# fverdoja/Fast-3D-Pointcloud-Segmentation

Hardware: AMD Instinct MI355X
Metric: Mpoints/sec segmented end-to-end, 1M-pt RGB-D frames (higher is better)
Workload: dtype f32

## Files before the change

__graft_entry__.py:

```python
import importlib
import os
import subprocess
import sys

ROOT = os.path.dirname(os.path.abspath(__file__))
PKG = "fast-3d-pointcloud-segmentation_amd"


def _run(cmd):
    print("+", " ".join(cmd), flush=True)
    subprocess.run(cmd, check=True)


def build() -> None:
    _run(["make", "-C", os.path.join(ROOT, PKG, "csrc")])
    _run(["make", "-C", os.path.join(ROOT, "oracle")])
    _run(["make", "-C", os.path.join(ROOT, "tests", "emul")])
    _run(["make", "-C", os.path.join(ROOT, "tests", "devprobe")])
    _run(["make", "-C", os.path.join(ROOT, "tests", "kernprobe")])
    _run(["make", "-C", os.path.join(ROOT, "tests", "blockprobe")])
    if ROOT not in sys.path:
        sys.path.insert(0, ROOT)
    P = importlib.import_module(PKG)
    lib = P.load_library()
    assert lib.f3ds_version() >= 120
    P.check_library_is_current(lib)


def smoke() -> None:
    import ctypes
    import numpy as np
    if ROOT not in sys.path:
        sys.path.insert(0, ROOT)
    sys.path.insert(0, os.path.join(ROOT, "tests"))
    P = importlib.import_module(PKG)
    from conftest import CpuChecker
    if P.device_count() < 1:
        raise RuntimeError("smoke(): no HIP device visible; libf3ds has no CPU fallback")
    pts = P.synth_frame(0, 7, 160, 120, 30)
    prm = P.launch_params(voxel_res=0.02, seed_res=0.2)
    ctx = P.Context(0)
    labels = ctx.segment(pts, prm)
    ora = CpuChecker(os.path.join(ROOT, "oracle", "libf3ds_oracle.so"), "f3ds_oracle")
    rc, olabels, ores, oh = ora.segment(pts, prm)
    assert rc == 0
    assert np.array_equal(labels, olabels), "HIP labels differ from the oracle"
    assert ctx.result.n_regions == ores.n_regions and ctx.result.n_merges == ores.n_merges
    print("smoke ok: N=%d V=%d S=%d E=%d merges=%d regions=%d  (%.2f ms on device 0)" % (
        len(pts), ctx.result.n_voxels, ctx.result.n_supervoxels, ctx.result.n_edges, ctx.result.n_merges, ctx.result.n_regions, ctx.result.ms_total))
    ctx.close()


if __name__ == "__main__":
    build()
    if len(sys.argv) > 1 and sys.argv[1] == "smoke":
        smoke()
```

fast-3d-pointcloud-segmentation_amd/__init__.py:

```python
import ctypes
import os

import numpy as np

_HERE = os.path.dirname(os.path.abspath(__file__))
def _dev_env(name):
    return os.environ.get(name) if os.environ.get("F3DS_DEV", "0") not in ("", "0") else None


LIB_PATH = _dev_env("F3DS_LIB") or os.path.join(_HERE, "libf3ds.so")

NO_LABEL = 0xFFFFFFFF
LAB_CIEDE00, RGB_EUCL = 0, 1
NORMALS_DIFF, CONVEX_NORMALS_DIFF = 0, 1
MANUAL_LAMBDA, ADAPTIVE_LAMBDA, EQUALIZATION = 0, 1, 2
DEPTH_U16, DEPTH_F32 = 0, 1
COLOR_RGB8, COLOR_RGBA8, COLOR_PACKED = 0, 1, 2

DBG = dict(GRID=0, VOXEL_KEYS=1, VOXEL_COUNT=2, VOXEL_XYZ=3, VOXEL_RGB=4, VOXEL_NORMAL=5, VOXEL_NEIGHBORS=6,
           POINT_VOXEL=7, SEED_ORIG=8, SEED_KEPT=9, VOXEL_SVLABEL=10, VOXEL_DIST=11, SV_LABELS=12, SV_CENTROID=13,
           EDGES=14, EDGE_DELTAS=15, EDGE_WEIGHTS=16, MERGES=17, VOXEL_REGION=18, SV_REGION=19)
DBG_INFO = dict(MERGE_LAYOUT=20, TILE_LIST_LEN=21, SWEEP_STATS=22, STAGE0_PATH=23, LAUNCH_SHAPE=24)
DBG_CLOUD_PATH = 25
DBG_DTYPE = dict(GRID=np.float64, VOXEL_KEYS=np.uint32, VOXEL_COUNT=np.uint32, VOXEL_XYZ=np.float32, VOXEL_RGB=np.float32,
                 VOXEL_NORMAL=np.float32, VOXEL_NEIGHBORS=np.int32, POINT_VOXEL=np.int32, SEED_ORIG=np.int32, SEED_KEPT=np.int32,
                 VOXEL_SVLABEL=np.uint32, VOXEL_DIST=np.float32, SV_LABELS=np.uint32, SV_CENTROID=np.float32, EDGES=np.uint32,
                 EDGE_DELTAS=np.float32, EDGE_WEIGHTS=np.float32, MERGES=np.uint32, VOXEL_REGION=np.uint32, SV_REGION=np.uint32)


class F3dsError(RuntimeError):
    def __init__(self, code, text):
        super().__init__("f3ds error %d: %s" % (code, text))
        self.code = code


class LogicError(F3dsError):
    """std::logic_error of the reference (clustering.cpp:576,591,671)."""


class Params(ctypes.Structure):
    _fields_ = [("voxel_res", ctypes.c_float), ("seed_res", ctypes.c_float), ("w_color", ctypes.c_float),
                ("w_spatial", ctypes.c_float), ("w_normal", ctypes.c_float), ("use_transform", ctypes.c_int32),
                ("color_metric", ctypes.c_int32), ("geom_metric", ctypes.c_int32), ("merging", ctypes.c_int32),
                ("lambda_", ctypes.c_float), ("bins", ctypes.c_int32), ("threshold", ctypes.c_float),
                ("leaf_order", ctypes.c_int32), ("fold_negative_z", ctypes.c_int32)]

    def copy(self):
        p = Params()
        ctypes.memmove(ctypes.byref(p), ctypes.byref(self), ctypes.sizeof(Params))
        return p


class Result(ctypes.Structure):
    _fields_ = [("n_points", ctypes.c_uint64), ("n_finite", ctypes.c_uint64), ("n_voxels", ctypes.c_uint32),
                ("octree_depth", ctypes.c_uint32), ("n_seed_cells", ctypes.c_uint32), ("n_seeds", ctypes.c_uint32),
                ("n_supervoxels", ctypes.c_uint32), ("n_edges", ctypes.c_uint32), ("n_merges", ctypes.c_uint32),
                ("n_regions", ctypes.c_uint32), ("sweeps", ctypes.c_uint32), ("lambda_", ctypes.c_float),
                ("ms_total", ctypes.c_float), ("ms_stage", ctypes.c_float * 8)]

    def as_dict(self):
        d = {k: getattr(self, k) for k, _ in self._fields_ if k != "ms_stage"}
        d["ms_stage"] = list(self.ms_stage)
        return d


class RgbdFormat(ctypes.Structure):
    _fields_ = [("width", ctypes.c_uint32), ("height", ctypes.c_uint32), ("depth_type", ctypes.c_int32), ("depth_scale", ctypes.c_float),
                ("color_format", ctypes.c_int32), ("depth_pitch", ctypes.c_uint32), ("color_pitch", ctypes.c_uint32),
                ("fx", ctypes.c_float), ("fy", ctypes.c_float), ("cx", ctypes.c_float), ("cy", ctypes.c_float)]

    def copy(self):
        f = RgbdFormat()
        ctypes.memmove(ctypes.byref(f), ctypes.byref(self), ctypes.sizeof(RgbdFormat))
        return f


# ... 952 lines not shown
        return self._get("region_adjacency", [_PAIR])[0]

    def cluster_supervoxels(self, sv, adjacency_pairs, params):
        a = {k: np.ascontiguousarray(sv[k], np.float32 if k in ("voxel_xyz", "centroid_xyz", "normal") else np.uint32) for k in
             ("label", "voxel_offset", "voxel_xyz", "voxel_rgba", "centroid_xyz", "normal")}
        S = len(a["label"])
        if a["voxel_offset"].shape != (S + 1,):
            raise ValueError("voxel_offset must hold n_supervoxels + 1 = %d entries, has shape %s" % (S + 1, a["voxel_offset"].shape))
        nvox = int(a["voxel_offset"][S])
        if a["voxel_xyz"].size != 3 * nvox or a["voxel_rgba"].size != nvox:
            raise ValueError("voxel_xyz / voxel_rgba must hold voxel_offset[-1] = %d voxels (have %d / %d)" % (nvox, a["voxel_xyz"].size // 3, a["voxel_rgba"].size))
        if a["centroid_xyz"].size != 3 * S or a["normal"].size != 3 * S:
            raise ValueError("centroid_xyz and normal must have shape (%d, 3)" % S)
        st = SupervoxelSet(S, *[a[k].ctypes.data for k in ("label", "voxel_offset", "voxel_xyz", "voxel_rgba", "centroid_xyz", "normal")])
        pairs = np.ascontiguousarray(adjacency_pairs, np.uint32).reshape(-1, 2)
        region = np.zeros(S, np.uint32); vlab = np.zeros(nvox, np.uint32)
        _check(self.lib, self.lib.f3ds_cluster_supervoxels(self.handle, ctypes.byref(st), pairs.ctypes.data, len(pairs), ctypes.byref(params), region.ctypes.data,
                                                           vlab.ctypes.data, ctypes.byref(self.result)))
        self._n = nvox
        return region, vlab

    def regions(self):
        return dict(zip(("label", "n_voxels", "xyz", "normal", "rgb"), self._get("regions", [_U32, _U32, _XYZ, _XYZ, _XYZ])))

    def region_voxels(self):
        return tuple(self._get("region_voxels", [_XYZ, _U32, _U32]))

    def voxel_cloud(self):
        return tuple(self._get("voxel_cloud", [_XYZ, _U32, _U32]))

    def merge_layout(self):
        nb = ctypes.c_size_t(); buf = np.zeros(2, np.uint32)
        _check(self.lib, self.lib.f3ds_get_debug(self.handle, 20, buf.ctypes.data, 8, ctypes.byref(nb)))
        return int(buf[0]), int(buf[1])

    def stage0_path(self):
        nb = ctypes.c_size_t(); buf = np.zeros(1, np.uint32)
        _check(self.lib, self.lib.f3ds_get_debug(self.handle, 23, buf.ctypes.data, 4, ctypes.byref(nb)))
        return "tiles" if buf[0] else "sort"

    def launch_shape(self):
        nb = ctypes.c_size_t(); buf = np.zeros(3, np.uint32)
        _check(self.lib, self.lib.f3ds_get_debug(self.handle, DBG_INFO["LAUNCH_SHAPE"], buf.ctypes.data, 12, ctypes.byref(nb)))
        return tuple(int(x) for x in buf)

    def sweep_stats(self):
        nb = ctypes.c_size_t(); buf = np.zeros(4, np.uint32)
        _check(self.lib, self.lib.f3ds_get_debug(self.handle, 22, buf.ctypes.data, 16, ctypes.byref(nb)))
        return tuple(int(x) for x in buf)

    def tile_list_lengths(self):
        return self._get("debug", [(np.uint8, ())], DBG_INFO["TILE_LIST_LEN"])[0].view(np.uint32)

    def debug(self, name):
        return self._get("debug", [(np.uint8, ())], DBG[name])[0].view(DBG_DTYPE[name])


class FrameStream(_Handle):

    _destroy = "f3ds_stream_destroy"

    def __init__(self, device=0, depth=8, groups=0):
        self.lib = load_library()
        h = ctypes.c_void_p()
        _check(self.lib, self.lib.f3ds_stream_create(device, depth, groups, ctypes.byref(h)))
        self.handle = h
        self.depth = depth

    def __enter__(self):
        return self

    def __exit__(self, *exc):
        self.close()

    def pending(self):
        return self.lib.f3ds_stream_pending(self.handle)

    def buffer(self, n):
        p = ctypes.c_void_p()
        rc = self.lib.f3ds_stream_buffer(self.handle, n, ctypes.byref(p))
        if rc == ERR_BUSY:
            return None
        _check(self.lib, rc)
        return np.ctypeslib.as_array(ctypes.cast(p, ctypes.POINTER(ctypes.c_float)), shape=(max(n, 1), 4))[:n]

    def submit(self, points, params, tag=0):
        pts = np.ascontiguousarray(points, np.float32).reshape(-1, 4)
        rc = self.lib.f3ds_stream_submit(self.handle, pts.ctypes.data, len(pts), ctypes.byref(params), tag)
        if rc == ERR_BUSY:
            return False
        _check(self.lib, rc)
        return True

    def submit_rgbd(self, depth, color, fmt, params, tag=0):
        f, d, c = _rgbd_images(fmt, depth, color)
        rc = self.lib.f3ds_stream_submit_rgbd(self.handle, ctypes.byref(f), d.ctypes.data, c.ctypes.data, ctypes.byref(params), tag)
        if rc == ERR_BUSY:
            return False
        _check(self.lib, rc)
        return True

    def next(self, wait=True):
        n = ctypes.c_size_t(); tag = ctypes.c_uint64(); res = Result()
        probe = np.empty(1, np.uint32)
        rc = self.lib.f3ds_stream_next(self.handle, probe.ctypes.data, 0, ctypes.byref(n), ctypes.byref(tag), ctypes.byref(res), 1 if wait else 0)
        if rc in (ERR_EMPTY, ERR_BUSY):
# ... 687 lines not shown
```

fast-3d-pointcloud-segmentation_amd/csrc/f3ds_algo.h:

```cpp
#ifndef F3DS_ALGO_H_
#define F3DS_ALGO_H_

#include "f3ds_numerics.h"

namespace f3ds {

#define F3DS_MAX_SEED_EVENTS 48
struct SeedEvent {
    int trigger;
    int depth;
    double min[3];
    unsigned off[3];
};
struct SeedGrid {
    int n_events;
    int error;
    int defined;
    int depth;
    double res;
    double min[3], max[3];
    unsigned off[3];
    SeedEvent ev[F3DS_MAX_SEED_EVENTS];
};
F3DS_HD void a_seed_init(SeedGrid& g, float seed_res) {
// ... 455 lines not shown
    rec[0] = acc[6] / c; rec[1] = acc[7] / c; rec[2] = acc[8] / c;
    float n4[4];
    n_plane_normal(acc, count, rec, n4);
    rec[3] = n4[0]; rec[4] = n4[1]; rec[5] = n4[2];
    rec[6] = acc[9]; rec[7] = acc[10]; rec[8] = acc[11];
    n_rgb2lab(rec + 6, rec + 9);
    rec[12] = rec[13] = rec[14] = rec[15] = 0.0f;
}

struct MergeParams {
    int color_metric, geom_metric, merging;
    float lambda;
    int bins;
    const float* cdf_c;
    const float* cdf_g;
};
F3DS_HD float a_tc(const MergeParams& p, float dc, int* err) {
    if (p.merging != 2) return p.lambda * dc;
    short bin = (short)__builtin_floorf(dc * (float)(short)p.bins);
    if (bin == (short)p.bins) bin--;
    if (bin < 0 || bin >= (short)p.bins) { *err = -9; return 0.0f; }
    return p.cdf_c[bin] / 2;
}
F3DS_HD float a_tg(const MergeParams& p, float dg, int* err) {
    if (p.merging != 2) return (1 - p.lambda) * dg;
    short bin = (short)__builtin_floorf(dg * (float)(short)p.bins);
    if (bin < 0 || bin >= (short)p.bins) { *err = -9; return 0.0f; }
    return p.cdf_g[bin] / 2;
}
template <class K = m_lit> F3DS_HD float a_edge_weight(const MergeParams& p, const float* rec_first, const float* rec_second, int* err, K mc = K()) {
    float dc, dg;
    n_delta_c_g(rec_first, rec_second, p.color_metric, p.geom_metric, &dc, &dg, mc);
    return a_tc(p, dc, err) + a_tg(p, dg, err);
}

struct EdgeHist {
    const uint32_t* ev_epoch;
    const uint32_t* ev_key;
    const int* ev_prev;
};
F3DS_HD bool a_edge_before(const EdgeHist& H, uint32_t e, uint32_t ke, int he, uint32_t f, uint32_t kf, int hf) {
    if (ke != kf) return ke < kf;
    for (;;) {
        uint32_t te = H.ev_epoch[he], tf = H.ev_epoch[hf];
        uint32_t tau = te > tf ? te : tf;
        if (tau == 0u) return e < f;
        if (te == tau) he = H.ev_prev[he];
        if (tf == tau) hf = H.ev_prev[hf];
        ke = H.ev_key[he]; kf = H.ev_key[hf];
        if (ke != kf) return ke < kf;
    }
}

}
#endif
```

fast-3d-pointcloud-segmentation_amd/csrc/f3ds_hip.hip:

```cpp
#include <hip/hip_runtime.h>

#include <algorithm>
#include <cmath>
#include <atomic>
#include <map>
#include <chrono>
#include <cstdio>
#include <cstdlib>
#include <cstring>
#include <string>
#include <type_traits>
#include <mutex>
#include <set>
#include <vector>

#include "../../include/f3ds.h"
#include "f3ds_algo.h"
#include "f3ds_glasbey.h"
#include "f3ds_eval.h"
#include "f3ds_dev.h"
#include "f3ds_levels.h"
#include "f3ds_eval_levels.h"
#include "f3ds_rgbd.h"
#include "f3ds_label_image.h"
// ... 1668 lines not shown
}

extern "C" int f3ds_get_supervoxels(f3ds_ctx* c, uint32_t* label, float* xyz, float* rgb, float* normal, uint32_t* n_voxels, size_t cap, size_t* n_out) {
    if (const int frc = on_frame(c)) return frc;
    return supervoxels_of(c, c->hcount, c->hc, label, xyz, rgb, normal, n_voxels, cap, n_out);
}

extern "C" int f3ds_get_supervoxel_adjacency(f3ds_ctx* c, uint32_t* pairs, size_t cap_pairs, size_t* n_out) {
    if (const int frc = on_frame(c)) return frc;
    const uint32_t E = c->E;
    int rc;
    if (!all_fit(E, cap_pairs, pairs != nullptr, n_out, &rc)) return rc;
    std::vector<uint32_t> a, b;
    if ((rc = fetch(c, c->ea0, E, a)) || (rc = fetch(c, c->eb0, E, b))) return rc;
    for (uint32_t e = 0; e < E; ++e) { pairs[2 * e] = label_out(c, a[e]); pairs[2 * e + 1] = label_out(c, b[e]); }
    return F3DS_OK;
}

extern "C" int f3ds_get_region_adjacency(f3ds_ctx* c, uint32_t* pairs, size_t cap_pairs, size_t* n_out) {
    if (const int frc = on_frame(c)) return frc;
    std::vector<uint32_t> a, b, root;
    int rc;
    if ((rc = fetch(c, c->ea0, c->E, a)) || (rc = fetch(c, c->eb0, c->E, b)) || (rc = fetch(c, c->root, c->S0 + 1, root))) return rc;
    std::vector<uint64_t> keys;
    for (uint32_t e = 0; e < c->E; ++e) {
        const uint32_t p = root[a[e]], q = root[b[e]];
        if (p != q) keys.push_back(((uint64_t)(p < q ? p : q) << 32) | (p < q ? q : p));
    }
    std::sort(keys.begin(), keys.end());
    keys.erase(std::unique(keys.begin(), keys.end()), keys.end());
    if (!all_fit(keys.size(), cap_pairs, pairs != nullptr, n_out, &rc)) return rc;
    for (size_t k = 0; k < keys.size(); ++k) { pairs[2 * k] = label_out(c, (uint32_t)(keys[k] >> 32)); pairs[2 * k + 1] = label_out(c, (uint32_t)keys[k]); }
    return F3DS_OK;
}

extern "C" int f3ds_merge_layout_info(uint32_t n_edges, int waves, int keys_in_lds, uint32_t out[4]) {
    if (!out || (waves != 4 && waves != 8) || (keys_in_lds != 0 && keys_in_lds != 2)) return F3DS_ERR_ARG;
    const MergeIlLayout L = merge_il_offsets(n_edges, waves, keys_in_lds);
    out[0] = L.total; out[1] = L.sp_rows; out[2] = L.Ecap;
    out[3] = (L.total <= MC_LDS_LIMIT && (uint64_t)n_edges * (keys_in_lds == 2 ? 10u : 2u) <= (1u << 22)) ? 1u : 0u;
    return F3DS_OK;
}
extern "C" int f3ds_get_debug(f3ds_ctx* c, int what, void* dst, size_t cap_bytes, size_t* bytes_out) {
    if (const int frc = on_frame(c, NEED_NOTHING)) return frc;
    const uint32_t V = c->V, S0 = c->S0, E = c->E, n = c->n;
    std::vector<uint8_t> buf;
    auto put = [&](const void* src, size_t nb) { const uint8_t* b = static_cast<const uint8_t*>(src); buf.insert(buf.end(), b, b + nb); };
    int rc = F3DS_OK;
    std::vector<float> f; std::vector<uint32_t> u, u2, u3; std::vector<int> iv; std::vector<unsigned char> uc;
    if (what != F3DS_DBG_GRID && what != F3DS_DBG_LAUNCH_SHAPE && what != F3DS_DBG_CLOUD_PATH && !c->have_frame) return F3DS_ERR_LOGIC;
    switch (what) {
        case F3DS_DBG_GRID: { HIPCHECK(hipMemcpy(c->h_grid, c->d_grid, sizeof(GridInfo), hipMemcpyDeviceToHost)); double g[5] = {c->h_grid->min[0], c->h_grid->min[1], c->h_grid->min[2], c->h_grid->res, (double)c->h_grid->depth}; put(g, sizeof g); break; }
        case F3DS_DBG_TILE_LIST_LEN: if ((rc = fetch(c, c->tile_n1, (size_t)(V + NT_TILE - 1) / NT_TILE, u))) return rc; put(u.data(), u.size() * 4); break;
        case F3DS_DBG_LAUNCH_SHAPE: put(c->launch_shape, 12); break;
        case F3DS_DBG_CLOUD_PATH: put(&c->cloud_path, 4); break;
        case F3DS_DBG_STAGE0_PATH: { const uint32_t w = c->vox_hashed ? 1u : 0u; put(&w, 4); break; }
        case F3DS_DBG_SWEEP_STATS: {
            DevCounters dcs;
            HIPCHECK(hipMemcpy(&dcs, c->d_dc, sizeof dcs, hipMemcpyDeviceToHost));
            put(dcs.sweep_stats, 16);
#ifdef F3DS_CEN_STATS
            fprintf(stderr, "d_centroid: quads %u, live rows %u, to the wave path: list %u, leaves %u; per quad ndmax %.2f, max leaves %.1f; per row nd %.2f, leaves %.1f\n", dcs.cen_stats[0], dcs.cen_stats[1], dcs.cen_stats[2],
                    dcs.cen_stats[3], dcs.cen_stats[4] / (double)dcs.cen_stats[0], dcs.cen_stats[7] / (double)dcs.cen_stats[0], dcs.cen_stats[5] / (double)dcs.cen_stats[1], dcs.cen_stats[6] / (double)dcs.cen_stats[1]);
#endif
            break;
        }
        case F3DS_DBG_MERGE_LAYOUT: { const uint32_t w[2] = {c->merge_kind == MK_GLOBAL ? 0u : (uint32_t)mk_waves(c->merge_kind), c->merge_kind == MK_GLOBAL ? 0u : (uint32_t)mk_res(c->merge_kind)}; put(w, 8); break; }
        case F3DS_DBG_VOXEL_KEYS: if ((rc = fetch(c, c->vkey, (size_t)V * 3, u))) return rc; put(u.data(), u.size() * 4); break;
        case F3DS_DBG_VOXEL_COUNT: if ((rc = fetch(c, c->vcount, V, u))) return rc; put(u.data(), u.size() * 4); break;
        case F3DS_DBG_VOXEL_XYZ: case F3DS_DBG_VOXEL_RGB: case F3DS_DBG_VOXEL_NORMAL:
            if ((rc = fetch(c, c->vf, (size_t)V * 12, f))) return rc;
            for (uint32_t v = 0; v < V; ++v) {
                if (what == F3DS_DBG_VOXEL_XYZ) put(&f[(size_t)v * 12], 12);
                else if (what == F3DS_DBG_VOXEL_RGB) put(&f[(size_t)v * 12 + 3], 12);
                else { float n4[4] = {f[(size_t)v * 12 + 6], f[(size_t)v * 12 + 7], f[(size_t)v * 12 + 8], 0.0f}; put(n4, 16); }
            }
            break;
        case F3DS_DBG_VOXEL_NEIGHBORS: if ((rc = fetch(c, c->nbr, (size_t)V * 27, iv))) return rc; put(iv.data(), iv.size() * 4); break;
        case F3DS_DBG_POINT_VOXEL: if ((rc = fetch(c, c->pt_voxel, n, iv))) return rc; put(iv.data(), iv.size() * 4); break;
        case F3DS_DBG_SEED_ORIG: if ((rc = fetch(c, c->seed_orig, c->C, iv))) return rc; put(iv.data(), iv.size() * 4); break;
        case F3DS_DBG_SEED_KEPT: if ((rc = fetch(c, c->seed_kept, S0, iv))) return rc; put(iv.data(), iv.size() * 4); break;
        case F3DS_DBG_VOXEL_SVLABEL: if ((rc = fetch(c, c->owner0, V, u))) return rc; put(u.data(), u.size() * 4); break;
        case F3DS_DBG_VOXEL_DIST: if ((rc = fetch(c, c->dist0, V, f))) return rc; put(f.data(), f.size() * 4); break;
        case F3DS_DBG_SV_LABELS: case F3DS_DBG_SV_CENTROID: case F3DS_DBG_SV_REGION:
            if ((rc = fetch(c, c->hcount, S0 + 1, u)) || (rc = fetch(c, c->hc, (size_t)(S0 + 1) * 12, f)) || (rc = fetch(c, c->root, S0 + 1, u2))) return rc;
            for (uint32_t h = 1; h <= S0; ++h) {
                if (!u[h]) continue;
                const uint32_t lh = label_out(c, h), lr = label_out(c, u2[h]);
                if (what == F3DS_DBG_SV_LABELS) put(&lh, 4);
                else if (what == F3DS_DBG_SV_REGION) put(&lr, 4);
                else { float r[10]; for (int k = 0; k < 9; ++k) r[k] = f[(size_t)h * 12 + k]; r[9] = 0.0f; put(r, 40); }
            }
            break;
        case F3DS_DBG_EDGES:
            if ((rc = fetch(c, c->ea0, E, u)) || (rc = fetch(c, c->eb0, E, u2))) return rc;
            for (uint32_t e = 0; e < E; ++e) { const uint32_t la = label_out(c, u[e]), lb = label_out(c, u2[e]); put(&la, 4); put(&lb, 4); }
            break;
        case F3DS_DBG_EDGE_DELTAS: if ((rc = fetch(c, c->deltas, (size_t)E * 2, f))) return rc; put(f.data(), f.size() * 4); break;
        case F3DS_DBG_EDGE_WEIGHTS: {
            if ((rc = fetch(c, c->deltas, (size_t)E * 2, f))) return rc;
            MergeParams mp; mp.color_metric = c->prm.color_metric; mp.geom_metric = c->prm.geom_metric; mp.merging = c->prm.merging;
            mp.lambda = c->res.lambda; mp.bins = (c->prm.merging == F3DS_EQUALIZATION && c->prm.bins != 0) ? (short)c->prm.bins : 500;
            std::vector<float> cdf;
            if (c->prm.merging == F3DS_EQUALIZATION) { if ((rc = fetch(c, c->cdf, (size_t)2 * mp.bins, cdf))) return rc; mp.cdf_c = cdf.data(); mp.cdf_g = cdf.data() + mp.bins; }
            else { mp.cdf_c = mp.cdf_g = nullptr; }
            for (uint32_t e = 0; e < E; ++e) { int err = 0; float w = a_tc(mp, f[e * 2], &err) + a_tg(mp, f[e * 2 + 1], &err); put(&w, 4); }
// ... 1067 lines not shown
```

fast-3d-pointcloud-segmentation_amd/csrc/f3ds_kernels.inc:

```


namespace {

struct P16 { float x, y, z; uint32_t rgba; };

struct DevCounters {
    unsigned long long n_finite;
    uint32_t bbox[6];
    uint32_t bbox_any;
    uint32_t n_valid;
    uint32_t n_voxels;
    uint32_t n_cells;
    uint32_t n_seeds;
    uint32_t n_edges;
    uint32_t n_alive;
    uint32_t n_merges;
    uint32_t n_regions;
    uint32_t n_events;
    int error;
    int r_overflow;
    float lambda;
    uint32_t seg_count;
    uint32_t n_ghosts;
    int depth;
// ... 1044 lines not shown
constexpr int SW_SLOT_BITS = 9;
constexpr int SW_SLOT_WORDS = (27 * SW_SLOT_BITS + 31) / 32;
static_assert(NT_RING1 < (1 << SW_SLOT_BITS), "a list position must fit its bit field");
__device__ __forceinline__ void sw_slots_pack(const uint32_t pos[27], uint32_t w[SW_SLOT_WORDS]) {
#pragma unroll
    for (int k = 0; k < SW_SLOT_WORDS; ++k) w[k] = 0u;
#pragma unroll
    for (int j = 0; j < 27; ++j) {
        const int bit = j * SW_SLOT_BITS, wi = bit >> 5, sh = bit & 31;
        w[wi] |= pos[j] << sh;
        if (sh + SW_SLOT_BITS > 32) w[wi + 1] |= pos[j] >> (32 - sh);
    }
}
__device__ __forceinline__ uint32_t sw_slot(const uint32_t w[SW_SLOT_WORDS], int j) {
    const int bit = j * SW_SLOT_BITS, wi = bit >> 5, sh = bit & 31;
    uint32_t x = w[wi] >> sh;
    if (sh + SW_SLOT_BITS > 32) x |= w[wi + 1] << (32 - sh);
    return x & ((1u << SW_SLOT_BITS) - 1u);
}
__device__ inline void cov_add(float acc[9], const float4 q) {
    acc[0] += q.x * q.x; acc[1] += q.x * q.y; acc[2] += q.x * q.z;
    acc[3] += q.y * q.y; acc[4] += q.y * q.z; acc[5] += q.z * q.z;
    acc[6] += q.x; acc[7] += q.y; acc[8] += q.z;
}
__device__ __forceinline__ uint32_t lds_addr(const float* p);
typedef float f3ds_f2 __attribute__((ext_vector_type(2)));
typedef float f3ds_f4 __attribute__((ext_vector_type(4)));
struct CovPairs {
    f3ds_f2 a0, a1, a2, a3; float sz;
    __device__ void zero() { a0 = a1 = a2 = a3 = f3ds_f2{0.0f, 0.0f}; sz = 0.0f; }
    __device__ void add(const f3ds_f4 q) {
        const f3ds_f2 xy = q.xy, zy = q.zw;
        a0 += xy * q.xx;
        a1 += xy * q.zz;
        a2 += zy * zy;
        a3 += xy;
        sz += q.z;
    }
    __device__ void store(float acc[9]) const { acc[0] = a0.x; acc[1] = a0.y; acc[2] = a1.x; acc[3] = a2.y; acc[4] = a1.y; acc[5] = a2.x; acc[6] = a3.x; acc[7] = a3.y; acc[8] = sz; }
};
template <int NTT>
struct d_normals_t {
    static constexpr int BLOCK = NTT;
    static constexpr int PT = (NT_RING1 * 27 + NTT - 1) / NTT;
    static constexpr int PR = PT % 9 == 0 ? 9 : (PT % 8 == 0 ? 8 : (PT % 6 == 0 ? 6 : (PT % 4 == 0 ? 4 : (PT % 3 == 0 ? 3 : (PT % 2 == 0 ? 2 : 1)))));
#ifndef F3DS_NORMALS_WPS
#define F3DS_NORMALS_WPS 3
#endif
#ifndef F3DS_NORMALS_WPS256
#define F3DS_NORMALS_WPS256 3
#endif
    static constexpr int WAVES_PER_SIMD = NTT > 256 ? F3DS_NORMALS_WPS : F3DS_NORMALS_WPS256;
    __device__ static uint32_t hslot(uint32_t ord) { return (ord * 2654435761u) >> 21; }
    __device__ void one_tile(const uint32_t bix, float* vf, const int* nbr, const DevCounters* dc, uint32_t* tile_n1, uint32_t* tile_ord, uint32_t* tile_slots, uint32_t holes) const {
        __shared__ uint32_t hw[NT_HCAP];
        __shared__ __attribute__((aligned(16))) float4 xyz[NT_SLOTS + 1];
        __shared__ uint32_t sord[NT_SLOTS];
        __shared__ uint16_t rows[NT_RING1 + 1][28];
        __shared__ uint32_t n_slots, overflow;
        __shared__ uint16_t tme[NT_TILE];
        const uint32_t KB = lds_addr(reinterpret_cast<const float*>(xyz)) >> 4;
        const uint32_t V = dc->n_voxels;
        const uint32_t v0 = bix * NT_TILE;
        if (v0 >= V) return;
        const uint32_t nt = V - v0 < (uint32_t)NT_TILE ? V - v0 : (uint32_t)NT_TILE;
#ifdef F3DS_MERGE_PROF
        unsigned long long tp[8], tq = __builtin_amdgcn_s_memtime(); int tpi = 0;
        unsigned long long tx_[12] = {0, 0, 0, 0, 0, 0, 0, 0, 0, 0, 0, 0}, tq2 = tq;
#define NPH() do { const unsigned long long n_ = __builtin_amdgcn_s_memtime(); tp[tpi++] = n_ - tq; tq = n_; } while (0)
#define NPX(i) do { const unsigned long long n_ = __builtin_amdgcn_s_memtime(); tx_[i] = n_ - tq2; tq2 = n_; } while (0)
#else
#define NPH() do { } while (0)
#define NPX(i) do { } while (0)
#endif
        for (int i = threadIdx.x; i < NT_HCAP; i += NTT) hw[i] = 0u;
        if (threadIdx.x == 0) { n_slots = 0; overflow = V >= NT_ORD_LIMIT ? 1u : 0u; xyz[NT_ZERO] = make_float4(0.0f, 0.0f, 0.0f, 0.0f); }
        __syncthreads();
        auto insert_key_from = [&](uint32_t ord, uint32_t h, uint32_t old) -> uint32_t {
            for (int probes = 0; probes < NT_HCAP; ++probes) {
                if (old == 0u) old = atomicCAS(&hw[h], 0u, ((ord + 1u) << 10) | NT_HNONE);
                if (old == 0u || (old >> 10) == ord + 1u) return h;
                h = (h + 1u) & (NT_HCAP - 1);
                old = hw[h];
            }
            overflow = 1;
            return 0u;
        };
        auto lookup = [&](uint32_t ord) -> uint16_t {
            uint32_t h = hslot(ord);
            for (;;) {
                const uint32_t k = hw[h];
                if ((k >> 10) == ord + 1u) return (k & NT_HNONE) == NT_HNONE ? NT_NONE : (uint16_t)(k & NT_HNONE);
                if (k == 0u) return NT_NONE;
                h = (h + 1u) & (NT_HCAP - 1);
            }
        };
        NPH();
        {
            constexpr int R1 = (NT_TILE * 27 + NTT - 1) / NTT;
            int u1[R1];
#pragma unroll
            for (int j = 0; j < R1; ++j) {
                const uint32_t t = threadIdx.x + (uint32_t)j * NTT;
                const uint32_t tt = t < nt * 27u ? t : 0u;
                u1[j] = nbr[(size_t)v0 * 27 + tt];
            }
            uint32_t h1[R1], o1[R1];
#pragma unroll
// ... 117 lines not shown
                }
                const float vp[3] = {self.x, self.y, self.z};
                float n4[4];
                n_plane_normal(acc, cnt, vp, n4);
                float* nout = vf + (size_t)v * 12 + 6;
                nout[0] = n4[0]; nout[1] = n4[1]; nout[2] = n4[2];
            }
            return;
        }
        const uint32_t ns = n_slots;
        for (uint32_t i = threadIdx.x; i < ns; i += NTT) { float4 q = *reinterpret_cast<const float4*>(vf + (size_t)sord[i] * 12); q.w = q.y; xyz[i] = q; }
#pragma unroll
        for (int j = 0; j < PT; ++j) {
            const uint32_t t = threadIdx.x + (uint32_t)j * NTT;
            if (t < n1 * 27u) {
                const uint32_t i = t / 27u, sl = t - i * 27u;
                const uint32_t pos = rows[i][sl];
                const uint32_t w = hw[pos != 0xFFFFu ? pos : 0u];
                rows[i][sl] = (uint16_t)((pos != 0xFFFFu ? (w & NT_HNONE) : (uint32_t)NT_ZERO) + KB);
            }
        }
        __syncthreads();
        {
            uint32_t* const stage_slots = hw;
            static_assert(SW_SLOT_WORDS * NT_TILE <= NT_HCAP, "the staged slot words fit the hash table's memory");
            const uint16_t ZBv = (uint16_t)(NT_ZERO + KB);
            for (uint32_t i = threadIdx.x; i < n1; i += NTT) {
                uint2 rw[7];
                const uint2* rp = reinterpret_cast<const uint2*>(&rows[i][0]);
#pragma unroll
                for (int k = 0; k < 7; ++k) rw[k] = rp[k];
                uint32_t ent[27];
#pragma unroll
                for (int j = 0; j < 27; ++j) { const uint32_t w = ((j >> 1) & 1) ? rw[j >> 2].y : rw[j >> 2].x; ent[j] = (j & 1) ? (w >> 16) : (w & 0xFFFFu); }
                const uint32_t ti = sord[i] - v0;
                if (ti < nt) {
                    uint32_t pos[27], pk[SW_SLOT_WORDS];
#pragma unroll
                    for (int j = 0; j < 27; ++j) { const uint32_t e = ent[j] - KB; pos[j] = e == NT_ZERO ? (uint32_t)NT_RING1 : e; }
                    sw_slots_pack(pos, pk);
#pragma unroll
                    for (int k = 0; k < SW_SLOT_WORDS; ++k) stage_slots[k * NT_TILE + ti] = pk[k];
                }
                uint16_t* const r = &rows[i][0];
                uint32_t w = 0;
#pragma unroll
                for (int j = 0; j < 27; ++j) if (ent[j] != (uint32_t)ZBv) { r[w] = (uint16_t)ent[j]; ++w; }
                for (uint32_t k = w; k < 27u; ++k) r[k] = ZBv;
                r[27] = (uint16_t)w;
            }
        }
        if (threadIdx.x < 28u) rows[NT_RING1][threadIdx.x] = threadIdx.x < 27u ? (uint16_t)(NT_ZERO + KB) : (uint16_t)0;
        __syncthreads();
        if (threadIdx.x == 0) tile_n1[bix] = (holes && bix % holes == 1u) ? SW_TILE_NONE : n1;
        for (uint32_t i = threadIdx.x; i < n1; i += NTT) tile_ord[(size_t)bix * NT_RING1 + i] = sord[i];
        for (uint32_t e = threadIdx.x; e < (uint32_t)(SW_SLOT_WORDS * NT_TILE); e += NTT) if ((e & (uint32_t)(NT_TILE - 1)) < nt) tile_slots[(size_t)bix * SW_SLOT_WORDS * NT_TILE + e] = hw[e];
        NPH();
#ifndef F3DS_NT_ACC_MODE
#define F3DS_NT_ACC_MODE 0
#endif
        const uint32_t wv = threadIdx.x >> 6;
        uint32_t ai = wv == 0u ? threadIdx.x : (wv == 2u ? threadIdx.x - 64u : 0xFFFFFFFFu);
        if (F3DS_NT_ACC_MODE == 1) ai = threadIdx.x - ((bix & 1u) ? 128u : 0u);
        if (F3DS_NT_ACC_MODE == 2) ai = wv == 0u ? threadIdx.x : (wv == 4u ? threadIdx.x - 192u : 0xFFFFFFFFu);
        if (F3DS_NT_ACC_MODE == 3) ai = threadIdx.x;
        if (F3DS_NT_ACC_MODE == 4) ai = (bix & 1u) ? (wv == 1u ? threadIdx.x - 64u : (wv == 3u ? threadIdx.x - 128u : 0xFFFFFFFFu)) : ai;
        if (ai >= nt) return;
        const uint32_t v = v0 + ai;
        const uint16_t me = tme[ai];
        CovPairs cp; cp.zero();
        unsigned cnt = 1;
        const f3ds_f4* xyz4 = reinterpret_cast<const f3ds_f4*>(xyz);
        const float4 self = xyz[me];
        cp.add(xyz4[me]);
        typedef uint32_t nt_u4 __attribute__((ext_vector_type(4)));
        typedef uint32_t nt_u2 __attribute__((ext_vector_type(2)));
#define NT_ROW_ISSUE(R, addr) asm volatile("ds_read2_b64 %0, %4 offset1:1\n\tds_read2_b64 %1, %4 offset0:2 offset1:3\n\tds_read2_b64 %2, %4 offset0:4 offset1:5\n\tds_read_b64 %3, %4 offset:48" \
            : "=&v"(R##a), "=&v"(R##b), "=&v"(R##c), "=&v"(R##d) : "v"(addr) : "memory")
#define NT_ROW_WORD(R, i) ((i) < 4 ? R##a[(i) & 3] : (i) < 8 ? R##b[(i) & 3] : (i) < 12 ? R##c[(i) & 3] : R##d[(i) & 1])
#define NT_C_ISSUE(cen_, addr) asm volatile("ds_read_b128 %0, %1" : "=v"(cen_) : "v"(addr) : "memory")
#define NT_U16_ISSUE(x, addr) asm volatile("ds_read_u16 %0, %1" : "=v"(x) : "v"(addr) : "memory")
#define NT_ENTRY_ADDR(a_, w_, hi_) do { if (hi_) asm volatile("v_lshlrev_b32_sdwa %0, %1, %2 dst_sel:DWORD dst_unused:UNUSED_PAD src0_sel:DWORD src1_sel:WORD_1" : "=v"(a_) : "v"(four), "v"(w_)); \
            else asm volatile("v_lshlrev_b32_sdwa %0, %1, %2 dst_sel:DWORD dst_unused:UNUSED_PAD src0_sel:DWORD src1_sel:WORD_0" : "=v"(a_) : "v"(four), "v"(w_)); } while (0)
#define NT_Q_ISSUE(Q, R, e_, b_) do { _Pragma("unroll") for (int k_ = 0; k_ < 7; ++k_) { const int j_ = 7 * (b_) + k_; uint32_t a_; \
            if (j_ == 0) a_ = (e_) << 4; else { const uint32_t w_ = NT_ROW_WORD(R, (j_ - 1) >> 1); NT_ENTRY_ADDR(a_, w_, (j_ - 1) & 1); } \
            NT_C_ISSUE(Q[k_], a_); } } while (0)
#define NT_Q_WAIT(Q, n) asm volatile("s_waitcnt lgkmcnt(" #n ")" : "+v"(Q[0]), "+v"(Q[1]), "+v"(Q[2]), "+v"(Q[3]), "+v"(Q[4]), "+v"(Q[5]), "+v"(Q[6]) :: "memory")
#define NT_ROW_WAIT(R, ent_, n) asm volatile("s_waitcnt lgkmcnt(" #n ")" : "+v"(R##a), "+v"(R##b), "+v"(R##c), "+v"(R##d), "+v"(ent_) :: "memory")
#define NT_ADD7(Q) do { _Pragma("unroll") for (int k_ = 0; k_ < 7; ++k_) cp.add(Q[k_]); } while (0)
#define NT_POSITION(RX, eX, RY, eY, eZ, zpos) do { \
            NT_Q_ISSUE(q1, RX, eX, 1); \
            NT_Q_WAIT(q0, 7); \
            cnt += ((eX) != ZB ? 1u : 0u) + (RX##d[1] >> 16); \
            NT_ADD7(q0); \
            NT_U16_ISSUE(eZ, myrow_a + 2u * (uint32_t)((zpos) < 27 ? (zpos) : 26)); \
            NT_ROW_ISSUE(RY, row_addr(eY)); \
            NT_Q_ISSUE(q0, RX, eX, 2); \
            NT_Q_WAIT(q1, 12); \
            NT_ADD7(q1); \
            NT_Q_ISSUE(q1, RX, eX, 3); \
            NT_Q_WAIT(q0, 7); \
            NT_ADD7(q0); \
            NT_ROW_WAIT(RY, eZ, 7); \
            NT_Q_ISSUE(q0, RY, eY, 0); \
            NT_Q_WAIT(q1, 7); \
            NT_ADD7(q1); } while (0)
        const uint32_t rows_a = lds_addr(reinterpret_cast<const float*>(&rows[0][0])), myrow_a = rows_a + (uint32_t)me * 56u;
        const uint32_t ZB = (uint32_t)NT_ZERO + KB;
        uint32_t four = 4u; asm volatile("" : "+v"(four));
        auto row_addr = [&](uint32_t e) { return rows_a + (e != ZB ? e - KB : (uint32_t)NT_RING1) * 56u; };
        const uint16_t* myrow = &rows[me][0];
        uint32_t eA = myrow[0], eB = myrow[1], eA2 = 0u, eB2 = 0u;
        nt_u4 RAa, RAb, RAc, RBa, RBb, RBc; nt_u2 RAd, RBd;
        f3ds_f4 q0[7], q1[7];
        asm volatile("s_waitcnt lgkmcnt(0)" : "+v"(eA), "+v"(eB) :: "memory");
        NT_ROW_ISSUE(RA, row_addr(eA));
        NT_ROW_WAIT(RA, eA, 0);
        NT_Q_ISSUE(q0, RA, eA, 0);
        uint32_t pmax = 0u;
        { const uint32_t mine_ = rows[me][27];
#pragma unroll
          for (uint32_t bit = 16u; bit; bit >>= 1) if (__ballot(mine_ >= (pmax | bit))) pmax |= bit; }
        const int phalf = (int)((pmax + 1u) >> 1);
#pragma unroll 1
        for (int p = 0; p < phalf; ++p) {
            if (2 * p + 1 >= 27) eB = ZB;
            NT_POSITION(RA, eA, RB, eB, eA2, 2 * p + 2);
            if (2 * p + 2 >= 27) eA2 = ZB;
            NT_POSITION(RB, eB, RA, eA2, eB2, 2 * p + 3);
            eA = eA2; eB = eB2;
        }
        NT_Q_WAIT(q0, 0);
#undef NT_ROW_ISSUE
#undef NT_ROW_WORD
#undef NT_ENTRY_ADDR
#undef NT_C_ISSUE
#undef NT_U16_ISSUE
#undef NT_Q_ISSUE
#undef NT_Q_WAIT
#undef NT_ROW_WAIT
#undef NT_ADD7
#undef NT_POSITION
        NPH();
        float acc[9];
        cp.store(acc);
        const float vp[3] = {self.x, self.y, self.z};
        float n4[4];
        n_plane_normal(acc, cnt, vp, n4);
        float* nout = vf + (size_t)v * 12 + 6;
        nout[0] = n4[0]; nout[1] = n4[1]; nout[2] = n4[2];
        NPH();
#ifdef F3DS_MERGE_PROF
        if (ai == 0u && f3ds_frame() == 0 && (bix == 10u || bix == 200u)) printf("d_normals tile %u, table phases: words+probes %llu | inserts %llu barrier %llu | numbering %llu barrier %llu | ring-2 words %llu | probes+inserts %llu barrier %llu | numbering %llu barrier %llu\n", bix, tx_[0], tx_[1], tx_[2], tx_[3], tx_[4], tx_[5], tx_[6], tx_[7], tx_[8], tx_[9]);
        if (ai == 0u && f3ds_frame() == 0 && (bix == 10u || bix == 200u)) printf("d_normals tile %u: init %llu ring1 %llu ring2 %llu rows+centroids %llu accumulate %llu normal %llu cycles (slots %u)\n", bix, tp[0], tp[1], tp[2], tp[3], tp[4], tp[5], ns);
#endif
#undef NPH
#undef NPX
    }
    __device__ void operator()(float* vf, const int* nbr, const DevCounters* dc, uint32_t* tile_n1, uint32_t* tile_ord, uint32_t* tile_slots, uint32_t holes) const {
        const uint32_t V = dc->n_voxels;
#ifdef F3DS_NORMALS_LOOP
        for (uint32_t b = BIX; b * (uint32_t)NT_TILE < V; b += gridDim.x) {
            one_tile(b, vf, nbr, dc, tile_n1, tile_ord, tile_slots, holes);
            __syncthreads();
        }
#else
        if (BIX * (uint32_t)NT_TILE < V) one_tile(BIX, vf, nbr, dc, tile_n1, tile_ord, tile_slots, holes);
#endif
    }
};

constexpr int SEED_CHUNK = 256;
struct d_chunkbox {
    static constexpr int BLOCK = SEED_CHUNK;
    __device__ void operator()(const float* vf, const DevCounters* dc, float* boxes) const {
        const uint32_t V = dc->n_voxels;
        const uint32_t v = BIX * SEED_CHUNK + threadIdx.x;
        if (BIX * SEED_CHUNK >= V) return;
        float mn[3] = {F3DS_FLT_MAX, F3DS_FLT_MAX, F3DS_FLT_MAX}, mx[3] = {-F3DS_FLT_MAX, -F3DS_FLT_MAX, -F3DS_FLT_MAX};
        if (v < V) { const float* p = vf + (size_t)v * 12; for (int a = 0; a < 3; ++a) { mn[a] = p[a]; mx[a] = p[a]; } }
        __shared__ float smn[SEED_CHUNK / 64][3], smx[SEED_CHUNK / 64][3];
    #pragma unroll
        for (int d = 32; d >= 1; d >>= 1)
            for (int a = 0; a < 3; ++a) {
                float t = __shfl_xor(mn[a], d, 64); if (t < mn[a]) mn[a] = t;
                t = __shfl_xor(mx[a], d, 64); if (t > mx[a]) mx[a] = t;
            }
        if (lane_id() == 0) for (int a = 0; a < 3; ++a) { smn[threadIdx.x >> 6][a] = mn[a]; smx[threadIdx.x >> 6][a] = mx[a]; }
        __syncthreads();
        if (threadIdx.x == 0) {
            for (int w = 1; w < SEED_CHUNK / 64; ++w)
                for (int a = 0; a < 3; ++a) { if (smn[w][a] < mn[a]) mn[a] = smn[w][a]; if (smx[w][a] > mx[a]) mx[a] = smx[w][a]; }
            for (int a = 0; a < 3; ++a) { boxes[BIX * 6 + a] = mn[a]; boxes[BIX * 6 + 3 + a] = mx[a]; }
        }
    }
};
struct d_seed_grow {
    static constexpr bool LATENCY_KERNEL = true;
    static constexpr int BLOCK = 256;
    __device__ void operator()(const float* vf, const float* boxes, DevCounters* dc, float seed_res, SeedGrid* out) const {
        __shared__ SeedGrid g;
        __shared__ uint32_t cursor;
        __shared__ uint32_t found;
        const uint32_t V = dc->n_voxels;
        const uint32_t C = (V + SEED_CHUNK - 1) / SEED_CHUNK;
        if (threadIdx.x == 0) { a_seed_init(g, seed_res); cursor = 0; }
        __syncthreads();
        for (;;) {
            if (threadIdx.x == 0) found = 0xFFFFFFFFu;
            __syncthreads();
            const uint32_t c0 = cursor / SEED_CHUNK;
            if (cursor >= V || g.error) break;
// ... 2607 lines not shown
```

include/f3ds.h:

```cpp
#ifndef F3DS_H_
#define F3DS_H_

#include <stddef.h>
#include <stdint.h>

#ifdef __cplusplus
extern "C" {
#endif

#define F3DS_VERSION 120

#define F3DS_NO_LABEL 0xFFFFFFFFu

#define F3DS_OK 0
#define F3DS_ERR_ARG (-1)
#define F3DS_ERR_NO_DEVICE (-2)
#define F3DS_ERR_HIP (-3)
#define F3DS_ERR_DEPTH (-4)
#define F3DS_ERR_LOGIC (-5)
#define F3DS_ERR_RANGE (-6)
#define F3DS_ERR_UNSUPPORTED (-7)
#define F3DS_ERR_IO (-8)
#define F3DS_ERR_EQ_BIN (-9)
#define F3DS_ERR_CAPACITY (-10)
// ... 260 lines not shown
    float cov[6];
    float eigenvalue[3];
    float normal[3];
    float axis[3];
    float plane_d;
    float curvature;
    uint32_t reserved;
} f3ds_cloud_region;
typedef struct f3ds_cloud_regions_result { uint32_t n_regions, n_nonempty; uint64_t n_labelled, n_clamped, n_inliers; } f3ds_cloud_regions_result;
int f3ds_cloud_regions_host(const void* points16, size_t n, const uint32_t* labels, uint32_t n_regions, const f3ds_cloud_params* params ,
                            f3ds_cloud_region* rows, f3ds_region_box* boxes , f3ds_cloud_regions_result* result );
int f3ds_cloud_regions(f3ds_ctx* ctx, const void* points16, size_t n, const uint32_t* labels, uint32_t n_regions, const f3ds_cloud_params* params,
                       int inputs_on_device, f3ds_cloud_region* rows, f3ds_region_box* boxes , int rows_on_device,
                       f3ds_cloud_regions_result* result );
int f3ds_cloud_regions_batch(f3ds_ctx** ctxs, int nctx, const void* const* points, const size_t* counts, const uint32_t* const* labels,
                             const uint32_t* n_regions, const f3ds_cloud_params* params, int inputs_on_device, f3ds_cloud_region* const* rows,
                             f3ds_region_box* const* boxes , int rows_on_device,
                             f3ds_cloud_regions_result* results, int* status);

int f3ds_recluster(f3ds_ctx* ctx, const f3ds_params* params, uint32_t* point_labels,
                   int labels_on_device, f3ds_result* result);

int f3ds_get_voxel_cloud(f3ds_ctx* ctx, float* xyz, uint32_t* label, uint32_t* rgba, size_t cap,
                         size_t* n_out);

enum {
    F3DS_DBG_GRID = 0,
    F3DS_DBG_VOXEL_KEYS = 1,
    F3DS_DBG_VOXEL_COUNT = 2,
    F3DS_DBG_VOXEL_XYZ = 3,
    F3DS_DBG_VOXEL_RGB = 4,
    F3DS_DBG_VOXEL_NORMAL = 5,
    F3DS_DBG_VOXEL_NEIGHBORS = 6,
    F3DS_DBG_POINT_VOXEL = 7,
    F3DS_DBG_SEED_ORIG = 8,
    F3DS_DBG_SEED_KEPT = 9,
    F3DS_DBG_VOXEL_SVLABEL = 10,
    F3DS_DBG_VOXEL_DIST = 11,
    F3DS_DBG_SV_LABELS = 12,
    F3DS_DBG_SV_CENTROID = 13,
    F3DS_DBG_EDGES = 14,
    F3DS_DBG_EDGE_DELTAS = 15,
    F3DS_DBG_EDGE_WEIGHTS = 16,
    F3DS_DBG_MERGES = 17,
    F3DS_DBG_VOXEL_REGION = 18,
    F3DS_DBG_SV_REGION = 19,
    F3DS_DBG_TILE_LIST_LEN = 21,
    F3DS_DBG_SWEEP_STATS = 22,
    F3DS_DBG_STAGE0_PATH = 23,
    F3DS_DBG_LAUNCH_SHAPE = 24,
    F3DS_DBG_MERGE_LAYOUT = 20
};
#define F3DS_DBG_CLOUD_PATH 25
int f3ds_get_debug(f3ds_ctx* ctx, int what, void* dst, size_t cap_bytes, size_t* bytes_out);
int f3ds_merge_layout_info(uint32_t n_edges, int waves, int keys_in_lds, uint32_t out[4]);


int f3ds_get_voxel_centroid_cloud(f3ds_ctx* ctx, float* xyz, uint32_t* rgba, uint32_t* sv_label, size_t cap, size_t* n_out);

int f3ds_get_supervoxels(f3ds_ctx* ctx, uint32_t* label, float* xyz, float* rgb, float* normal, uint32_t* n_voxels,
                         size_t cap, size_t* n_out);

int f3ds_get_supervoxel_adjacency(f3ds_ctx* ctx, uint32_t* pairs, size_t cap_pairs, size_t* n_out);

int f3ds_get_region_adjacency(f3ds_ctx* ctx, uint32_t* pairs, size_t cap_pairs, size_t* n_out);

typedef struct f3ds_supervoxel_set {
    uint32_t n_supervoxels;
    const uint32_t* label;
    const uint32_t* voxel_offset;
    const float* voxel_xyz;
    const uint32_t* voxel_rgba;
    const float* centroid_xyz;
    const float* normal;
} f3ds_supervoxel_set;
int f3ds_cluster_supervoxels(f3ds_ctx* ctx, const f3ds_supervoxel_set* sv, const uint32_t* adjacency_pairs, size_t n_pairs,
                             const f3ds_params* params, uint32_t* region_of_sv, uint32_t* voxel_labels, f3ds_result* result);

int f3ds_get_regions(f3ds_ctx* ctx, uint32_t* label, uint32_t* n_voxels, float* centroid_xyz, float* normal, float* mean_rgb,
                     size_t cap, size_t* n_out);
int f3ds_get_region_voxels(f3ds_ctx* ctx, float* xyz, uint32_t* rgba, uint32_t* voxel_index, size_t cap, size_t* n_out);

typedef struct f3ds_performance { float voi, precision, recall, fscore, wov, fpr, fnr; } f3ds_performance;

int f3ds_evaluate(f3ds_ctx* ctx, const uint32_t* truth_point_labels, f3ds_performance* out);

int f3ds_auto_threshold(f3ds_ctx* ctx, const f3ds_params* params, const uint32_t* truth_point_labels,
                        float start, float end, float step, float* thresholds, f3ds_performance* scores,
                        size_t cap, size_t* n_out, float* best_threshold, f3ds_performance* best_score,
                        uint32_t* point_labels, int labels_on_device, f3ds_result* result);

int f3ds_labels_at_thresholds(f3ds_ctx* ctx, const float* thresholds, int k, uint32_t* point_labels, int labels_on_device,
                              uint32_t* n_regions );
int f3ds_labels_at_thresholds_batch(f3ds_ctx** ctxs, int nctx, const float* thresholds, int k, uint32_t* const* point_labels,
                                    int labels_on_device, uint32_t* n_regions );
int f3ds_evaluate_levels(f3ds_ctx* ctx, const uint32_t* truth_point_labels, int truth_on_device, const float* thresholds, int k,
                         f3ds_performance* scores , uint32_t* n_regions );
int f3ds_evaluate_levels_batch(f3ds_ctx** ctxs, int nctx, const uint32_t* const* truth_point_labels, int truth_on_device,
                               const float* thresholds, int k, f3ds_performance* scores, uint32_t* n_regions);
int f3ds_best_level(const float* thresholds, const f3ds_performance* scores, int k, int* best_index);

int f3ds_get_merge_tree(f3ds_ctx* ctx, uint32_t* survivor, uint32_t* absorbed, float* weight, size_t cap, size_t* n_out);

int f3ds_refine_supervoxels(f3ds_ctx* ctx, int num_itr);
int f3ds_get_refined_voxels(f3ds_ctx* ctx, uint32_t* sv_label, float* normal, size_t cap, size_t* n_out);
int f3ds_get_refined_supervoxels(f3ds_ctx* ctx, uint32_t* label, float* xyz, float* rgb, float* normal, uint32_t* n_voxels,
// ... 44 lines not shown
```

Before: 3759.

## Renumber tile neighbor lists own-voxels-first and hand writeback to an idle wave

```diff
diff --git a/__graft_entry__.py b/__graft_entry__.py
--- a/__graft_entry__.py
+++ b/__graft_entry__.py
@@ -19,6 +19,7 @@
     _run(["make", "-C", os.path.join(ROOT, "tests", "devprobe")])
     _run(["make", "-C", os.path.join(ROOT, "tests", "kernprobe")])
     _run(["make", "-C", os.path.join(ROOT, "tests", "blockprobe")])
+    _run(["make", "-C", os.path.join(ROOT, "tests", "tileprobe")])
     if ROOT not in sys.path:
         sys.path.insert(0, ROOT)
     P = importlib.import_module(PKG)
diff --git a/fast-3d-pointcloud-segmentation_amd/__init__.py b/fast-3d-pointcloud-segmentation_amd/__init__.py
--- a/fast-3d-pointcloud-segmentation_amd/__init__.py
+++ b/fast-3d-pointcloud-segmentation_amd/__init__.py
@@ -22,6 +22,8 @@
            EDGES=14, EDGE_DELTAS=15, EDGE_WEIGHTS=16, MERGES=17, VOXEL_REGION=18, SV_REGION=19)
 DBG_INFO = dict(MERGE_LAYOUT=20, TILE_LIST_LEN=21, SWEEP_STATS=22, STAGE0_PATH=23, LAUNCH_SHAPE=24)
 DBG_CLOUD_PATH = 25
+DBG_TILE_ORD, DBG_TILE_SLOTS = 26, 27
+TILE_RING1 = 448
 DBG_DTYPE = dict(GRID=np.float64, VOXEL_KEYS=np.uint32, VOXEL_COUNT=np.uint32, VOXEL_XYZ=np.float32, VOXEL_RGB=np.float32,
                  VOXEL_NORMAL=np.float32, VOXEL_NEIGHBORS=np.int32, POINT_VOXEL=np.int32, SEED_ORIG=np.int32, SEED_KEPT=np.int32,
                  VOXEL_SVLABEL=np.uint32, VOXEL_DIST=np.float32, SV_LABELS=np.uint32, SV_CENTROID=np.float32, EDGES=np.uint32,
@@ -1080,6 +1082,18 @@
     def tile_list_lengths(self):
         return self._get("debug", [(np.uint8, ())], DBG_INFO["TILE_LIST_LEN"])[0].view(np.uint32)
 
+    def tile_lists(self):
+        o = self._get("debug", [(np.uint8, ())], DBG_TILE_ORD)[0].view(np.uint32).reshape(-1, TILE_RING1)
+        w = self._get("debug", [(np.uint8, ())], DBG_TILE_SLOTS)[0].view(np.uint32).reshape(-1, 8, 128).astype(np.uint64)
+        pos = np.empty((w.shape[0], 128, 27), np.uint32)
+        for j in range(27):
+            k, sh = divmod(9 * j, 32)
+            x = w[:, k, :] >> np.uint64(sh)
+            if sh + 9 > 32:
+                x = x | (w[:, k + 1, :] << np.uint64(32 - sh))
+            pos[:, :, j] = (x & np.uint64(511)).astype(np.uint32)
+        return o, pos
+
     def debug(self, name):
         return self._get("debug", [(np.uint8, ())], DBG[name])[0].view(DBG_DTYPE[name])
 
diff --git a/fast-3d-pointcloud-segmentation_amd/csrc/f3ds_algo.h b/fast-3d-pointcloud-segmentation_amd/csrc/f3ds_algo.h
--- a/fast-3d-pointcloud-segmentation_amd/csrc/f3ds_algo.h
+++ b/fast-3d-pointcloud-segmentation_amd/csrc/f3ds_algo.h
@@ -531,5 +531,13 @@
     }
 }
 
+F3DS_HD uint32_t a_tile_slot_own(uint32_t below, uint32_t a) { return below + a; }
+F3DS_HD uint32_t a_tile_slot_other(const uint32_t* others, uint32_t m, uint32_t k, uint32_t v0, uint32_t nt) {
+    uint32_t c = k > v0 ? nt : 0u;
+    for (uint32_t j = 0; j < m; j += 4u)
+        c += (others[j] < k ? 1u : 0u) + (others[j + 1u] < k ? 1u : 0u) + (others[j + 2u] < k ? 1u : 0u) + (others[j + 3u] < k ? 1u : 0u);
+    return c;
+}
+
 }
 #endif
diff --git a/fast-3d-pointcloud-segmentation_amd/csrc/f3ds_hip.hip b/fast-3d-pointcloud-segmentation_amd/csrc/f3ds_hip.hip
--- a/fast-3d-pointcloud-segmentation_amd/csrc/f3ds_hip.hip
+++ b/fast-3d-pointcloud-segmentation_amd/csrc/f3ds_hip.hip
@@ -1744,6 +1744,8 @@
     switch (what) {
         case F3DS_DBG_GRID: { HIPCHECK(hipMemcpy(c->h_grid, c->d_grid, sizeof(GridInfo), hipMemcpyDeviceToHost)); double g[5] = {c->h_grid->min[0], c->h_grid->min[1], c->h_grid->min[2], c->h_grid->res, (double)c->h_grid->depth}; put(g, sizeof g); break; }
         case F3DS_DBG_TILE_LIST_LEN: if ((rc = fetch(c, c->tile_n1, (size_t)(V + NT_TILE - 1) / NT_TILE, u))) return rc; put(u.data(), u.size() * 4); break;
+        case F3DS_DBG_TILE_ORD: if ((rc = fetch(c, c->tile_ord, (size_t)((V + NT_TILE - 1) / NT_TILE) * NT_RING1, u))) return rc; put(u.data(), u.size() * 4); break;
+        case F3DS_DBG_TILE_SLOTS: if ((rc = fetch(c, c->tile_slots, (size_t)((V + NT_TILE - 1) / NT_TILE) * SW_SLOT_WORDS * NT_TILE, u))) return rc; put(u.data(), u.size() * 4); break;
         case F3DS_DBG_LAUNCH_SHAPE: put(c->launch_shape, 12); break;
         case F3DS_DBG_CLOUD_PATH: put(&c->cloud_path, 4); break;
         case F3DS_DBG_STAGE0_PATH: { const uint32_t w = c->vox_hashed ? 1u : 0u; put(&w, 4); break; }
diff --git a/fast-3d-pointcloud-segmentation_amd/csrc/f3ds_kernels.inc b/fast-3d-pointcloud-segmentation_amd/csrc/f3ds_kernels.inc
--- a/fast-3d-pointcloud-segmentation_amd/csrc/f3ds_kernels.inc
+++ b/fast-3d-pointcloud-segmentation_amd/csrc/f3ds_kernels.inc
@@ -1120,8 +1120,8 @@
 #endif
     static constexpr int WAVES_PER_SIMD = NTT > 256 ? F3DS_NORMALS_WPS : F3DS_NORMALS_WPS256;
     __device__ static uint32_t hslot(uint32_t ord) { return (ord * 2654435761u) >> 21; }
-    __device__ void one_tile(const uint32_t bix, float* vf, const int* nbr, const DevCounters* dc, uint32_t* tile_n1, uint32_t* tile_ord, uint32_t* tile_slots, uint32_t holes) const {
-        __shared__ uint32_t hw[NT_HCAP];
+    __device__ __forceinline__ void one_tile(const uint32_t bix, float* vf, const int* nbr, const DevCounters* dc, uint32_t* tile_n1, uint32_t* tile_ord, uint32_t* tile_slots, uint32_t holes) const {
+        __shared__ __attribute__((aligned(16))) uint32_t hw[NT_HCAP];
         __shared__ __attribute__((aligned(16))) float4 xyz[NT_SLOTS + 1];
         __shared__ uint32_t sord[NT_SLOTS];
         __shared__ uint16_t rows[NT_RING1 + 1][28];
@@ -1345,19 +1345,69 @@
         }
         if (threadIdx.x < 28u) rows[NT_RING1][threadIdx.x] = threadIdx.x < 27u ? (uint16_t)(NT_ZERO + KB) : (uint16_t)0;
         __syncthreads();
-        if (threadIdx.x == 0) tile_n1[bix] = (holes && bix % holes == 1u) ? SW_TILE_NONE : n1;
-        for (uint32_t i = threadIdx.x; i < n1; i += NTT) tile_ord[(size_t)bix * NT_RING1 + i] = sord[i];
-        for (uint32_t e = threadIdx.x; e < (uint32_t)(SW_SLOT_WORDS * NT_TILE); e += NTT) if ((e & (uint32_t)(NT_TILE - 1)) < nt) tile_slots[(size_t)bix * SW_SLOT_WORDS * NT_TILE + e] = hw[e];
         NPH();
 #ifndef F3DS_NT_ACC_MODE
 #define F3DS_NT_ACC_MODE 0
 #endif
+        auto acc_lane = [&](uint32_t tid) -> uint32_t {
+            const uint32_t w = tid >> 6;
+            uint32_t a = w == 0u ? tid : (w == 2u ? tid - 64u : 0xFFFFFFFFu);
+            if (F3DS_NT_ACC_MODE == 1) a = tid - ((bix & 1u) ? 128u : 0u);
+            if (F3DS_NT_ACC_MODE == 2) a = w == 0u ? tid : (w == 4u ? tid - 192u : 0xFFFFFFFFu);
+            if (F3DS_NT_ACC_MODE == 3) a = tid;
+            if (F3DS_NT_ACC_MODE == 4) a = (bix & 1u) ? (w == 1u ? tid - 64u : (w == 3u ? tid - 128u : 0xFFFFFFFFu)) : a;
+            return a;
+        };
         const uint32_t wv = threadIdx.x >> 6;
-        uint32_t ai = wv == 0u ? threadIdx.x : (wv == 2u ? threadIdx.x - 64u : 0xFFFFFFFFu);
-        if (F3DS_NT_ACC_MODE == 1) ai = threadIdx.x - ((bix & 1u) ? 128u : 0u);
-        if (F3DS_NT_ACC_MODE == 2) ai = wv == 0u ? threadIdx.x : (wv == 4u ? threadIdx.x - 192u : 0xFFFFFFFFu);
-        if (F3DS_NT_ACC_MODE == 3) ai = threadIdx.x;
-        if (F3DS_NT_ACC_MODE == 4) ai = (bix & 1u) ? (wv == 1u ? threadIdx.x - 64u : (wv == 3u ? threadIdx.x - 128u : 0xFFFFFFFFu)) : ai;
+        const uint32_t ai = acc_lane(threadIdx.x);
+        uint32_t tw = 0;
+        while (tw < (uint32_t)(NTT / 64 - 1) && acc_lane(tw * 64u) < nt) ++tw;
+        if (wv == tw) {
+            uint32_t* const oth = hw + SW_SLOT_WORDS * NT_TILE;
+            uint16_t* const newpos = reinterpret_cast<uint16_t*>(oth + NT_RING1);
+            static_assert(NT_RING1 % 64 == 0 && SW_SLOT_WORDS * NT_TILE + NT_RING1 + (NT_RING1 + 2) / 2 <= NT_HCAP, "the renumbering scratch fits behind the staged slot words");
+            static_assert(NT_ORD_LIMIT <= (1u << (32 - SW_SLOT_BITS)), "an ordinal and a list position share a word");
+            constexpr int Q = NT_RING1 / 64;
+            const uint32_t lane = threadIdx.x & 63u;
+#pragma unroll
+            for (int q = 0; q < Q; ++q) oth[lane + 64u * q] = 0xFFFFFFFFu;
+            uint32_t m = 0, below = 0;
+#pragma unroll
+            for (int q = 0; q < Q; ++q) {
+                const uint32_t i = lane + 64u * q;
+                const uint32_t k = sord[i < n1 ? i : 0u];
+                const bool other = i < n1 && k - v0 >= nt;
+                const uint64_t b = __ballot(other);
+                if (other) oth[m + (uint32_t)__popcll(b & lanemask_lt())] = (k << SW_SLOT_BITS) | i;
+                below += (uint32_t)__popcll(__ballot(other && k < v0));
+                m += (uint32_t)__popcll(b);
+            }
+            __builtin_amdgcn_wave_barrier();
+            uint32_t* const ord_out = tile_ord + (size_t)bix * NT_RING1;
+#pragma unroll
+            for (int q = 0; q < Q; ++q) {
+                const uint32_t i = lane + 64u * q;
+                const uint32_t k = sord[i < n1 ? i : 0u];
+                if (i < n1 && k - v0 < nt) { const uint32_t r = a_tile_slot_own(below, k - v0); newpos[i] = (uint16_t)r; ord_out[r] = k; }
+            }
+            for (uint32_t x = lane; x < m; x += 64u) {
+                const uint32_t pk = oth[x], r = a_tile_slot_other(oth, m, pk, v0 << SW_SLOT_BITS, nt);
+                newpos[pk & ((1u << SW_SLOT_BITS) - 1u)] = (uint16_t)r; ord_out[r] = pk >> SW_SLOT_BITS;
+            }
+            if (lane == 0u) newpos[NT_RING1] = (uint16_t)NT_RING1;
+            __builtin_amdgcn_wave_barrier();
+            for (uint32_t t = lane; t < nt; t += 64u) {
+                uint32_t w[SW_SLOT_WORDS], pos[27], pk[SW_SLOT_WORDS];
+#pragma unroll
+                for (int k = 0; k < SW_SLOT_WORDS; ++k) w[k] = hw[k * NT_TILE + t];
+#pragma unroll
+                for (int j = 0; j < 27; ++j) pos[j] = newpos[sw_slot(w, j)];
+                sw_slots_pack(pos, pk);
+#pragma unroll
+                for (int k = 0; k < SW_SLOT_WORDS; ++k) tile_slots[(size_t)bix * SW_SLOT_WORDS * NT_TILE + k * NT_TILE + t] = pk[k];
+            }
+            if (lane == 0u) tile_n1[bix] = (holes && bix % holes == 1u) ? SW_TILE_NONE : n1;
+        }
         if (ai >= nt) return;
         const uint32_t v = v0 + ai;
         const uint16_t me = tme[ai];
@@ -1450,7 +1500,7 @@
 #undef NPH
 #undef NPX
     }
-    __device__ void operator()(float* vf, const int* nbr, const DevCounters* dc, uint32_t* tile_n1, uint32_t* tile_ord, uint32_t* tile_slots, uint32_t holes) const {
+    __device__ __forceinline__ void operator()(float* vf, const int* nbr, const DevCounters* dc, uint32_t* tile_n1, uint32_t* tile_ord, uint32_t* tile_slots, uint32_t holes) const {
         const uint32_t V = dc->n_voxels;
 #ifdef F3DS_NORMALS_LOOP
         for (uint32_t b = BIX; b * (uint32_t)NT_TILE < V; b += gridDim.x) {
diff --git a/include/f3ds.h b/include/f3ds.h
--- a/include/f3ds.h
+++ b/include/f3ds.h
@@ -336,6 +336,8 @@
     F3DS_DBG_MERGE_LAYOUT = 20
 };
 #define F3DS_DBG_CLOUD_PATH 25
+#define F3DS_DBG_TILE_ORD 26
+#define F3DS_DBG_TILE_SLOTS 27
 int f3ds_get_debug(f3ds_ctx* ctx, int what, void* dst, size_t cap_bytes, size_t* bytes_out);
 int f3ds_merge_layout_info(uint32_t n_edges, int waves, int keys_in_lds, uint32_t out[4]);
 
```

New measurement: 3719. 0.989x the previous value.
